# pangenome/povu

Measured on AMD Instinct MI355X. Metric: edges/sec decomposed (flubble+PVST), higher is better.
Workload: dtype u32

## Files before the change

include/povu_hip.h:

```cpp
#ifndef POVU_HIP_H
#define POVU_HIP_H

#include <stddef.h>
#include <stdint.h>

#ifdef __cplusplus
extern "C" {
#endif

#define POVU_HIP_NIL 0xFFFFFFFFu
#define POVU_SIDE_L 0
#define POVU_SIDE_R 1
#define POVU_TIP_NONE 0
#define POVU_TIP_L 1
#define POVU_TIP_R 2

typedef struct povu_hip_ctx povu_hip_ctx;
typedef struct povu_hip_forest povu_hip_forest;

int povu_hip_device_count(void);

povu_hip_ctx *povu_hip_create(int device, char *err, size_t errlen);
void povu_hip_destroy(povu_hip_ctx *ctx);
int povu_hip_release_workspace(povu_hip_ctx *ctx);
// ... 563 lines not shown
typedef struct {
	char name[48];
	double ms;
	uint32_t launches;
} povu_hip_stage_time;
int povu_hip_last_stage_times(const povu_hip_ctx *ctx, povu_hip_stage_time *out, int max);
typedef struct { char name[24]; int resident; uint64_t bytes; } povu_hip_arena_info;
int povu_hip_arena_report(const povu_hip_ctx *ctx, povu_hip_arena_info *out, int max);
uint32_t povu_hip_last_seq_redo(const povu_hip_ctx *ctx);
int povu_hip_last_black_only_classes(const povu_hip_ctx *ctx);
int povu_hip_last_narrow_counts(const povu_hip_ctx *ctx);
int povu_hip_last_prefix_records(const povu_hip_ctx *ctx);
uint64_t povu_hip_wide_repeats(const povu_hip_ctx *ctx);
int povu_hip_last_laminar_check_ran(const povu_hip_ctx *ctx);
int povu_hip_last_crossings(povu_hip_ctx *ctx, uint32_t out[2]);
uint64_t povu_hip_last_links_processed(const povu_hip_ctx *ctx);

int povu_hip_debug_components(povu_hip_ctx *ctx, uint32_t *comp_of, uint32_t *local_idx);
int povu_hip_debug_tree(povu_hip_ctx *ctx, uint32_t comp, uint32_t *n_tree, uint32_t *gid, uint8_t *typ,
			uint32_t *par, uint32_t *cls);
int povu_hip_debug_edge_ids(povu_hip_ctx *ctx, uint32_t comp, uint32_t *n_tree, uint32_t *tree_edge_id);
int povu_hip_debug_walk_words(povu_hip_ctx *ctx, uint32_t out[3]);
int povu_hip_debug_stack(povu_hip_ctx *ctx, uint32_t comp, uint32_t *n, uint32_t *tree_vtx, uint32_t *cls,
			 uint32_t *next_seen);

int povu_hip_debug_csr(povu_hip_ctx *ctx, uint32_t *off, uint32_t *adj, uint32_t *aoth, uint32_t *atwin, uint8_t *tip,
		       uint32_t words[4]);
#define POVU_HIP_ROWB_IDENTITY 1u
#define POVU_HIP_ROWB_SORT_FREE 2u
#define POVU_HIP_ROWB_LEAN_IDENTITY 4u
// ... 66 lines not shown
```

povu_amd/csrc/hip/common.hpp:

```cpp
#pragma once
#include <hip/hip_runtime.h>

#include "forest_wire.hpp"

#include <algorithm>
#include <cstdint>
#include <cstdio>
#include <cstring>
#include <stdexcept>
#include <string>
#include <vector>

#define POVU_NIL 0xFFFFFFFFu

__device__ __forceinline__ uint4 load4_unaligned(const unsigned *__restrict__ p)
{
	typedef unsigned v4a __attribute__((ext_vector_type(4), aligned(4)));
	const v4a v = *reinterpret_cast<const v4a *>(p);
	return make_uint4(v.x, v.y, v.z, v.w);
}

#define POVU_W2(v) "+v"((v).x), "+v"((v).y)
#define POVU_W4(v) "+v"((v).x), "+v"((v).y), "+v"((v).z), "+v"((v).w)
__device__ __forceinline__ void landed(uint32_t &a, uint32_t &b, uint32_t &c, uint32_t &d) { asm volatile("" : "+v"(a), "+v"(b), "+v"(c), "+v"(d)); }
__device__ __forceinline__ void landed(uint32_t &a, uint32_t &b, uint32_t &c, uint32_t &d, uint32_t &e)
{
	asm volatile("" : "+v"(a), "+v"(b), "+v"(c), "+v"(d), "+v"(e));
}
__device__ __forceinline__ void landed(uint2 &a, uint2 &b, uint2 &c, uint2 &d, uint32_t &e, uint32_t &f, uint32_t &g, uint32_t &h)
{
	asm volatile("" : POVU_W2(a), POVU_W2(b), POVU_W2(c), POVU_W2(d), "+v"(e), "+v"(f), "+v"(g), "+v"(h));
}
__device__ __forceinline__ void landed(uint4 &a, uint2 &b) { asm volatile("" : POVU_W4(a), POVU_W2(b)); }
__device__ __forceinline__ void landed(uint4 &a, uint4 &b, uint4 &c, uint4 &d) { asm volatile("" : POVU_W4(a), POVU_W4(b), POVU_W4(c), POVU_W4(d)); }
#define POVU_A2(a, W) W((a)[0]), W((a)[1])
#define POVU_A4(a, W) POVU_A2(a, W), W((a)[2]), W((a)[3])
#define POVU_A8(a, W) POVU_A4(a, W), W((a)[4]), W((a)[5]), W((a)[6]), W((a)[7])
#define POVU_W1(v) "+v"(v)
template <uint32_t N>
__device__ __forceinline__ void landed(uint32_t (&a)[N], uint32_t (&b)[N], uint32_t (&c)[N], uint32_t (&d)[N], uint32_t (&e)[N])
{
	static_assert(N == 2 || N == 4 || N == 8, "a batch of 2, 4 or 8");
	if constexpr (N == 2)
		asm volatile("" : POVU_A2(a, POVU_W1), POVU_A2(b, POVU_W1), POVU_A2(c, POVU_W1), POVU_A2(d, POVU_W1), POVU_A2(e, POVU_W1));
	else if constexpr (N == 4)
		asm volatile("" : POVU_A4(a, POVU_W1), POVU_A4(b, POVU_W1), POVU_A4(c, POVU_W1), POVU_A4(d, POVU_W1), POVU_A4(e, POVU_W1));
	else
		asm volatile("" : POVU_A8(a, POVU_W1), POVU_A8(b, POVU_W1), POVU_A8(c, POVU_W1), POVU_A8(d, POVU_W1), POVU_A8(e, POVU_W1));
// ... 563 lines not shown
```

povu_amd/csrc/hip/par_kernels.hip:

```cpp
#include "par_kernels.hpp"
#include "segtree.hpp"

#include <algorithm>
#include <cstdlib>
#include <type_traits>

namespace povu_hip
{

#define NIL POVU_NIL
static constexpr size_t PVST_STAGE_MIN = size_t(1) << 20;

__global__ void k_tcomp_vertices(uint32_t V, uint32_t T, const uint32_t *__restrict__ ckey, const uint32_t *__restrict__ voff,
				 uint32_t *__restrict__ t_comp)
{
	uint32_t i = BIDX * blockDim.x + threadIdx.x;
	if (i >= V)
		return;
	uint32_t c = ckey[i];
	t_comp[2 * i + c] = c;
	t_comp[2 * i + 1 + c] = c;
	if (i + 1 == voff[c + 1])
		t_comp[2 * i + 2 + c] = c;
	if (i == V - 1)
// ... 107 lines not shown
	__device__ __forceinline__ uint32_t operator()(uint32_t t) const
	{
		if (t_root)
			return t_root[t];
		uint32_t lo = 0, hi = C;
		while (hi - lo > 1) {
			const uint32_t mid = (lo + hi) >> 1;
			if (2 * voff[mid] + mid <= t)
				lo = mid;
			else
				hi = mid;
		}
		return 2 * voff[lo] + lo;
	}
};
__device__ __forceinline__ void capping_of(uint32_t v, const uint32_t *__restrict__ gsize, const uint32_t *__restrict__ hi0,
					   const uint4 *__restrict__ brec, const RootOf &root_of,
					   const SegTree &segA, uint32_t *__restrict__ cap_tgt,
					   uint8_t *__restrict__ capf, uint32_t *__restrict__ literal_rule_seen)
{
	const uint32_t end = v + gsize[v];
	uint32_t root = NIL;
	auto hi_of = [&](uint32_t c) {
		const uint32_t cs = max(gsize[c], 1u);
		if (bitrank(brec, c + cs) != bitrank(brec, c)) {
			if (root == NIL)
				root = root_of(v);
			return root;
		}
		if (cs <= 8) {
			uint32_t m = NIL;
			for (uint32_t k = c; k < c + cs; k++)
				m = min(m, hi0[k]);
			return m;
		}
		return seg_min(segA, c, c + cs);
	};
	uint32_t hi_1 = NIL, hi_child = NIL, lt_c[2] = {NIL, NIL}, lt_h[2] = {NIL, NIL};
	uint32_t second = NIL;
	for (uint32_t c = v + 1; c < end; c += max(gsize[c], 1u)) {
		const uint32_t h = hi_of(c);
		if (h < hi_1 || hi_child == NIL) {
			second = hi_1;
			hi_1 = h;
			hi_child = c;
		} else {
			second = min(second, h);
		}
		if (h < v) {
			if (lt_c[0] == NIL)
				lt_c[0] = c, lt_h[0] = h;
			else if (lt_c[1] == NIL)
				lt_c[1] = c, lt_h[1] = h;
		}
	}
	const uint32_t hi_2 = lt_c[0] != hi_child ? lt_h[0] : lt_h[1];
	if (hi_2 != (second < v ? second : NIL))
		*literal_rule_seen = 1u;
	if (hi_2 < hi0[v]) {
		cap_tgt[v] = hi_2;
		capf[v] = 1;
	}
}
static constexpr uint32_t HS_ITER = LIST_ITER, HS_VERTS = LIST_SPAN;
static_assert(TPB == (int)LIST_TPB, "append_in_order is written for workgroups of 256");
__global__ void __launch_bounds__(TPB) k_hi_simp(uint32_t T, const uint32_t *__restrict__ gsize, const uint4 *__restrict__ brec,
						  uint8_t *__restrict__ simp, uint8_t *__restrict__ hpf,
						  uint8_t *__restrict__ capf, uint32_t *__restrict__ br_list, uint32_t *__restrict__ n_br)
{
	const uint32_t B0 = BIDX * HS_VERTS;
	auto one = [&](uint32_t t, uint32_t sz, uint32_t br, uint32_t p0, uint32_t sz_next, uint32_t &sm, uint32_t &bch) {
		sm = (sz && br && bitrank(brec, t + sz) - p0 == 1) ? 1u : 0u;
		bch = (sz > 2 && t + 1 + max(sz_next, 1u) < t + sz) ? 1u : 0u;
	};
// ... 28 lines not shown
				simp[t] = (uint8_t)sm;
				if (t == T - 1)
					simp[T] = 0;
				if (hpf)
					hpf[t] = (uint8_t)sm;
				capf[t] = 0;
				b4 |= bch << (t - t0);
			}
		}
		bw |= (unsigned long long)b4 << (4 * it);
	}
	append_in_order(bw, B0, br_list, n_br);
}
__global__ void k_capping(const uint32_t *__restrict__ n_list, const uint32_t *__restrict__ list, const uint32_t *__restrict__ gsize,
			  const uint32_t *__restrict__ hi0, const uint4 *__restrict__ brec, const RootOf root_of, const SegTree segA,
			  uint32_t *__restrict__ cap_tgt, uint8_t *__restrict__ capf, uint32_t *__restrict__ literal_rule_seen)
{
	const uint32_t n = *n_list;
	for (uint32_t i = BIDX * blockDim.x + threadIdx.x; i < n; i += gridDim.x * blockDim.x)
		capping_of(list[i], gsize, hi0, brec, root_of, segA, cap_tgt, capf, literal_rule_seen);
}
static constexpr uint32_t BX_TILE = TPB;
__global__ void __launch_bounds__(TPB) k_flag_tile_counts(uint32_t T, const uint8_t *__restrict__ capf, const uint8_t *__restrict__ simp,
							   uint32_t *__restrict__ tcap, uint32_t *__restrict__ tsimp, uint32_t ntiles)
{
	const uint32_t e0 = (blockIdx.x * TPB + threadIdx.x) * 16u;
	uint32_t nc = 0, ns = 0;
	if (e0 + 16 <= T) {
		const uint4 a = *reinterpret_cast<const uint4 *>(capf + e0), b = *reinterpret_cast<const uint4 *>(simp + e0);
		const uint32_t wa[4] = {a.x, a.y, a.z, a.w}, wb[4] = {b.x, b.y, b.z, b.w};
#pragma unroll
		for (int k = 0; k < 4; k++)
#pragma unroll
			for (int q = 0; q < 4; q++) {
				nc += ((wa[k] >> (8 * q)) & 0xFFu) ? 1u : 0u;
// ... 153 lines not shown
	uint32_t i = BIDX * blockDim.x + threadIdx.x;
	if (i < n)
		dst[i] = src[idx[i]];
}
struct StackPlace {
	const uint32_t *voff, *soff, *shift;
	uint32_t *s_vtx;
};
template <bool BLACK, class PS, class BS>
__global__ void k_top_bracket(uint32_t n, const uint32_t *__restrict__ gsize, const uint32_t *__restrict__ gpar,
			      const uint32_t *__restrict__ mpre, const BS bstart,
			      const SegTree segB, const uint32_t *__restrict__ tgtR,
			      const PS psin, uint32_t *__restrict__ ckey, uint32_t *__restrict__ cval,
			      uint32_t *__restrict__ lsz, uint32_t *__restrict__ err, const uint32_t *__restrict__ rid,
			      uint32_t first_simp_id, uint8_t *__restrict__ hpf, const uint32_t *__restrict__ seg_comp,
			      const uint32_t *__restrict__ c_ntree, const StackPlace sp)
{
	const uint32_t q = BIDX * blockDim.x + threadIdx.x;
	if (q >= n)
		return;
	uint32_t v = n - 1 - q, c = 0;
	const uint32_t g = v;
	if (BLACK) {
		c = seg_comp[g];
		v = 2 * g + c + (c_ntree[c] & 1u) + 1;
	}
	uint32_t sz = gsize[v];
	if (sz == 0 || (!BLACK && gpar[v] == NIL)) {
		cval[q] = v;
		ckey[q] = NIL;
		if (!BLACK)
			lsz[v] = 0;
		return;
	}
	uint32_t at = v;
	if (BLACK) {
		at = sp.soff[c] + (g - sp.voff[c]) + sp.shift[g];
		sp.s_vtx[at] = v;
	}
	cval[q] = at;
	uint32_t m = mpre[v];
	uint32_t lo = bstart.at(m), hi = bstart.at(m + sz);
	const uint32_t live = (hi - lo) - (psin.at(v + sz) - psin.at(v));
	uint32_t i = NIL;
	if (live >= 1 && live <= 4) {
		const uint4 a = load4_unaligned(tgtR + (hi - live));
		const bool all = a.x < v && (live < 2 || a.y < v) && (live < 3 || a.z < v) && (live < 4 || a.w < v);
		if (all)
			i = hi - live;
	}
	if (i == NIL) {
		const uint32_t np = min(hi - lo, 4u);
		const uint4 a = load4_unaligned(tgtR + lo);
		if (np > 0 && a.x < v)
			i = lo;
		else if (np > 1 && a.y < v)
			i = lo + 1;
		else if (np > 2 && a.z < v)
			i = lo + 2;
		else if (np > 3 && a.w < v)
			i = lo + 3;
		if (i == NIL && lo + np < hi)
			i = seg_first_less(segB, lo + np, hi, v);
	}
	if (i == NIL) {
		atomicAdd(&err[PW_NO_BRACKET], 1u);
		ckey[q] = NIL;
		lsz[at] = 0;
		return;
	}
	lsz[at] = live;
	ckey[q] = i;
	if (hpf && rid[i] >= first_simp_id)
		hpf[v] |= 2;
}
template <bool BLACK>
__global__ void k_class_flags(uint32_t n, uint32_t V, const uint32_t *__restrict__ skey, const uint32_t *__restrict__ sval,
			      const uint32_t *__restrict__ lsz, const uint8_t *__restrict__ tf, uint8_t *__restrict__ flag,
			      uint32_t *__restrict__ dlt, uint32_t *__restrict__ mark)
{
	uint32_t q = BIDX * blockDim.x + threadIdx.x;
	if (!BLACK && q < V + 2)
		dlt[q] = 0;
	if (q >= n)
		return;
	uint32_t k = skey[q];
// ... 65 lines not shown
		return;
	const uint32_t p = lastb[q];
	if (!p)
		return;
	const uint32_t u = sval[q], d = sval[p - 1];
	if (gcls[u] != gcls[d])
		return;
	const uint32_t iu = sidx[u], id = sidx[d];
	ns[iu] = id;
	prev[id] = iu;
}

static constexpr uint32_t DF_OPENS = 1u, DF_SEEN = 2u;
__global__ void k_class_finish_black(uint32_t n, uint32_t S, const uint32_t *__restrict__ skey, const uint32_t *__restrict__ sval,
				     const uint32_t *__restrict__ lsz, uint8_t *__restrict__ flag, uint32_t *__restrict__ ns,
				     uint32_t *__restrict__ prev, bool write_prev, uint8_t *__restrict__ dflag)
{
	const uint32_t q0 = (BIDX * blockDim.x + threadIdx.x) * 4u;
	if (q0 == 0)
		dflag[S] = 0;
	if (q0 >= n)
		return;
	uint32_t K[6], U[6], L[6];
	if (q0 + 4 <= n) {
		const uint4 k4 = *reinterpret_cast<const uint4 *>(skey + q0), u4 = *reinterpret_cast<const uint4 *>(sval + q0);
		K[1] = k4.x, K[2] = k4.y, K[3] = k4.z, K[4] = k4.w;
		U[1] = u4.x, U[2] = u4.y, U[3] = u4.z, U[4] = u4.w;
	} else {
		for (uint32_t j = 1; j <= 4; j++) {
			K[j] = q0 + j - 1 < n ? skey[q0 + j - 1] : NIL;
			U[j] = q0 + j - 1 < n ? sval[q0 + j - 1] : 0u;
		}
	}
	K[0] = q0 ? skey[q0 - 1] : NIL, U[0] = q0 ? sval[q0 - 1] : 0u;
	K[5] = q0 + 4 < n ? skey[q0 + 4] : NIL, U[5] = q0 + 4 < n ? sval[q0 + 4] : 0u;
#pragma unroll
	for (int j = 0; j < 6; j++)
		L[j] = K[j] != NIL ? lsz[U[j]] : 0u;
	bool fresh[6];
	fresh[0] = true;
#pragma unroll
	for (int j = 1; j < 6; j++)
		fresh[j] = (q0 + j - 1 == 0) || K[j - 1] != K[j] || L[j - 1] != L[j];
	uint32_t fw = 0;
#pragma unroll
	for (int j = 1; j <= 4; j++) {
		const uint32_t q = q0 + j - 1;
		if (q >= n || K[j] == NIL)
			continue;
		const uint32_t u = U[j];
		fw |= (fresh[j] ? 1u : 0u) << (8 * (j - 1));
		const uint32_t nx = fresh[j] ? u : U[j - 1];
		ns[u] = nx;
		const bool seen = K[j + 1] != NIL && !fresh[j + 1];
		if (write_prev)
			prev[u] = seen ? U[j + 1] : NIL;
		dflag[u] = (uint8_t)(((u + 1 < nx) ? DF_OPENS : 0u) | (seen ? DF_SEEN : 0u));
	}
	if (q0 + 4 <= n) {
		*reinterpret_cast<uint32_t *>(flag + q0) = fw;
	} else {
		for (uint32_t j = 0; q0 + j < n; j++)
			flag[q0 + j] = (uint8_t)((fw >> (8 * j)) & 0xFFu);
	}
}
__global__ void k_class_ids_black(uint32_t n, const uint32_t *__restrict__ skey, const uint32_t *__restrict__ sval,
				  const uint8_t *__restrict__ fresh, const uint32_t *__restrict__ ps, uint32_t *__restrict__ s_cls)
{
	uint32_t q = BIDX * blockDim.x + threadIdx.x;
	if (q < n && skey[q] != NIL)
		s_cls[sval[q]] = ps[q] + fresh[q] - 1;
}
__global__ void k_cls_from_stack(uint32_t S, const uint32_t *__restrict__ s_vtx, const uint32_t *__restrict__ s_cls,
				 uint32_t *__restrict__ gcls)
{
	uint32_t i = BIDX * blockDim.x + threadIdx.x;
	if (i < S)
		gcls[s_vtx[i]] = s_cls[i];
}
__device__ __forceinline__ void laminar_check_one(uint32_t i, uint32_t p, const uint32_t *__restrict__ prev, const SegTree &segP,
						   uint8_t *__restrict__ xflag)
{
	if (p == NIL || p + 1 >= i)
		return;
	uint32_t lowest;
	if (i - p <= 9) {
// ... 513 lines not shown
	ParWs &pw;
	StageTimer &tm;
	hipStream_t s;
	const SideStream &side;
	PassTail &tail;
	const std::function<void *(size_t)> &alloc_result_block;
	const ClassViews v;
	const uint32_t C, V, T, S, n_processed;
	const int64_t dense_nb0;
	const bool dense;
	const bool want_hp;
	const bool lean;
	const bool narrow_oc, narrow_sc, narrow_ic;
	const int word_prefix;
	const bool rec_ps, rec_bs;
	bool black_only = false;
	const RootOf root_of;
	uint32_t NB0 = 0, ncap = 0, nsimp = 0, NB = 0, NC = 0;
	const uint32_t ntiles;
	uint32_t *extra = nullptr;
	HostScratch::Token extra_ready = 0;
	uint32_t *early = nullptr;
	HostScratch::Token early_ready = 0;
	bool use_side = false;

	ClassPass(const CompState &cs_, SeqWs &sw_, ParWs &pw_, uint32_t C_, uint32_t n_processed_, uint32_t n_stack, int64_t dense_nb0_,
		  const std::function<void *(size_t)> &alloc, StageTimer &tm_, hipStream_t s_, const SideStream &side_, PassTail &tail_)
		: cs(cs_), sw(sw_), pw(pw_), tm(tm_), s(s_), side(side_), tail(tail_), alloc_result_block(alloc), v(class_views(pw_)), C(C_),
		  V(sw_.V), T(2 * sw_.V + C_), S(n_stack), n_processed(n_processed_), dense_nb0(dense_nb0_), dense(dense_nb0_ >= 0),
		  want_hp(sw_.hairpins != nullptr), lean(dense && !want_hp), narrow_oc(dense && pw_.narrow_ordcnt),
		  narrow_sc(narrow_oc && pw_.narrow_srccnt), narrow_ic(narrow_sc && pw_.narrow_incnt),
		  word_prefix(getenv("POVU_HIP_WORD_PREFIX") ? atoi(getenv("POVU_HIP_WORD_PREFIX")) : 0), rec_ps(narrow_ic && word_prefix != 1 && word_prefix != 2),
		  rec_bs(narrow_sc && word_prefix != 1 && word_prefix != 3), root_of{lean ? nullptr : pw_.t_root, cs_.voff, C_},
		  ntiles((T + BX_TILE - 1) / BX_TILE)
	{
	}
	void scan(const uint32_t *in, uint32_t *out, size_t n) const { scan_exclusive_u32(in, out, n, pw.scan_tmp, pw.scan_tmp_bytes, s); }
	void scan8(const uint8_t *in, uint32_t *out, size_t n) const
	{
		scan_exclusive_u8(in, out, n, nullptr, nullptr, 0, pw.scan_tmp, pw.scan_tmp_bytes, s);
	}
	void scan8pair(const uint8_t *in0, uint32_t *out0, size_t n0, const uint8_t *in1, uint32_t *out1, size_t n1) const
	{
		scan_exclusive_u8(in0, out0, n0, in1, out1, n1, pw.scan_tmp, pw.scan_tmp_bytes, s);
	}
	uint4 *psin_rec() const { return reinterpret_cast<uint4 *>(pw.psin); }
	uint4 *bstart_rec() const { return reinterpret_cast<uint4 *>(v.bstart); }
	template <class F>
// ... 60 lines not shown
	seg_build(pw.segA, pw.hi0, T, s);
	if (P.narrow_ic)
		scan_exclusive_diff_u8_u8(pw.ordcnt8, pw.incnt8, v.pscov, (size_t)T + 1, pw.scan_tmp, pw.scan_tmp_bytes, s);
	else if (P.narrow_oc)
		scan_exclusive_diff_u8_u32(pw.ordcnt8, pw.incnt, v.pscov, (size_t)T + 1, pw.scan_tmp, pw.scan_tmp_bytes, s);
	else if (P.dense)
		scan_exclusive_diff_u32(pw.lsz, pw.incnt, v.pscov, (size_t)T + 1, pw.scan_tmp, pw.scan_tmp_bytes, s);
	else
		P.scan(pw.cov, v.pscov, (size_t)T + 1);
	KLAUNCH(k_bridge_flags, dim3(nblk(((size_t)T / 256 + 1) * 64)), dim3(TPB), 0, s, T, pw.gsize, P.sw.t_flags, v.pscov, v.brec);
	bitrank_build(v.brec, (size_t)T / 64 + 1, v.brec_cnt, pw.scan_tmp, pw.scan_tmp_bytes, s);
	uint32_t *n_br = pw.err + PW_N_BRIDGE;
	KLAUNCH(k_hi_simp, dim3((unsigned)(((size_t)T + HS_VERTS - 1) / HS_VERTS)), dim3(TPB), 0, s, T, pw.gsize, v.brec, v.simp, P.want_hp ? pw.hpf : nullptr, v.capf, v.br_list,
		n_br);
	KLAUNCH(k_capping, dim3(std::min<unsigned>(nblk(T / 8 + 1), 16384)), dim3(TPB), 0, s, n_br, v.br_list, pw.gsize, pw.hi0, v.brec, P.root_of,
		pw.segA, pw.cap_tgt, v.capf, pw.err + PW_LITERAL_RULE);
	KLAUNCH(k_flag_tile_counts, dim3((ntiles + 1 + 15) / 16 + 1), dim3(TPB), 0, s, T, v.capf, v.simp, v.tcap, v.tsimp, ntiles);
	scan_exclusive_u32_pair(v.tsimp, v.tsimp, (size_t)ntiles + 1, v.tcap, v.tcap, (size_t)ntiles + 1, pw.scan_tmp, pw.scan_tmp_bytes, s);
	if (!P.narrow_ic)
		publish_extra(P);
}

static bool place_brackets(ClassPass &P)
{
	ParWs &pw = P.pw;
	const ClassViews &v = P.v;
	hipStream_t s = P.s;
	const uint32_t T = P.T;
	auto bracket_extra = [&](auto *ordcnt, auto *sc, auto *ic) {
		using OC = std::remove_const_t<std::remove_pointer_t<decltype(ordcnt)>>;
		using SC = std::remove_pointer_t<decltype(sc)>;
// ... 79 lines not shown
{
	ParWs &pw = P.pw;
	const ClassViews &v = P.v;
	const CompState &cs = P.cs;
	hipStream_t s = P.s;
	const uint32_t V = P.V, NC = P.NC;
	uint32_t *sdl = pw.dlt;
	if (pw.sdl_filled && P.dense) {
		sdl = pw.sdl;
	} else {
		HIP_CHECK(hipMemsetAsync(pw.dlt, 0, ((size_t)V + 2) * 4, s));
		LAUNCH(k_shift_delta, V, s, V, cs.ckey, P.sw.c_ntree, pw.gsize, pw.dlt);
	}
	scan_inclusive_u32(sdl, v.shift_ps, (size_t)V + 1, pw.scan_tmp, pw.scan_tmp_bytes, s);
	const StackPlace sp{cs.voff, pw.soff, v.shift_ps, pw.s_vtx};
	P.with_prefix_views([&](auto ps, auto bs) {
		LAUNCH((k_top_bracket<true, decltype(ps), decltype(bs)>), NC, s, NC, pw.gsize, pw.gpar, pw.mpre, bs, pw.segB, pw.tgtR, ps, v.ck,
		       pw.vals_t, pw.lsz, pw.err, pw.b_val2, P.NB0 + P.ncap, nullptr, cs.ckey, P.sw.c_ntree, sp);
	});
	sort_pairs_u32(v.ck, v.ck2, pw.vals_t, pw.vals_t2, NC, bits_for((uint64_t)P.NB + 1), pw.sort_tmp, pw.sort_tmp_bytes, s);
	P.tm.end(30 + 2 * 22);
	P.tm.begin("par_stack");
	LAUNCH(k_class_finish_black, std::max<size_t>(((size_t)NC + 3) / 4, 1), s, NC, P.S, v.ck2, pw.vals_t2, pw.lsz, v.cflag, pw.ns, pw.prev,
	       pw.check_laminar, v.dflag);
	P.tm.end(1);
	P.tm.begin("par_next_seen");
	P.tm.end(0);
	pw.gcls_valid = false;
	pw.s_cls_valid = false;
}

static void classes_all_vertices(ClassPass &P)
{
	ParWs &pw = P.pw;
	const ClassViews &v = P.v;
	const CompState &cs = P.cs;
	const SeqWs &sw = P.sw;
	hipStream_t s = P.s;
	const uint32_t V = P.V, T = P.T, NC = P.NC;
	const StackPlace none{nullptr, nullptr, nullptr, nullptr};
	P.with_prefix_views([&](auto ps, auto bs) {
		LAUNCH((k_top_bracket<false, decltype(ps), decltype(bs)>), NC, s, NC, pw.gsize, pw.gpar, pw.mpre, bs, pw.segB, pw.tgtR, ps, v.ck,
		       pw.vals_t, pw.lsz, pw.err, pw.b_val2, P.NB0 + P.ncap, P.want_hp ? pw.hpf : nullptr, nullptr, nullptr, none);
	});
	sort_pairs_u32(v.ck, v.ck2, pw.vals_t, pw.vals_t2, NC, bits_for((uint64_t)P.NB + 1), pw.sort_tmp, pw.sort_tmp_bytes, s);
	LAUNCH(k_class_flags<false>, std::max<size_t>(NC, (size_t)V + 2), s, NC, V, v.ck2, pw.vals_t2, pw.lsz, sw.t_flags, v.cflag, pw.dlt,
	       v.mark);
	P.scan8(v.cflag, v.cps, (size_t)NC + 1);
	LAUNCH(k_class_scatter, NC, s, NC, v.ck2, pw.vals_t2, v.cflag, v.cps, pw.gcls);
	pw.gcls_valid = true;
	pw.s_cls_valid = true;
	P.tm.end(30 + 2 * 22);

	P.tm.begin("par_stack");
	LAUNCH(k_shift_delta, V, s, V, cs.ckey, sw.c_ntree, pw.gsize, pw.dlt);
	P.scan(pw.dlt, pw.dlt_ps, (size_t)V + 1);
	LAUNCH(k_stack_emit, V, s, V, cs.ckey, sw.c_ntree, cs.voff, pw.soff, pw.dlt, pw.dlt_ps, pw.gsize, pw.gcls, pw.s_vtx, pw.s_cls,
	       pw.topi, pw.ns, pw.prev);
// ... 154 lines not shown
	else
		classes_all_vertices(P);
	stack_directories(P);
	laminar_and_levels(P);
	emit_and_copy(P);
	return true;
}

static void stack_class_ids(ParWs &pw, hipStream_t s)
{
	if (pw.s_cls_valid)
		return;
	const uint32_t V = pw.V;
	const ClassViews v = class_views(pw);
	scan_exclusive_u8(v.cflag, v.cps, (size_t)V + 1, nullptr, nullptr, 0, pw.scan_tmp, pw.scan_tmp_bytes, s);
	LAUNCH(k_class_ids_black, V, s, V, v.ck2, pw.vals_t2, v.cflag, v.cps, pw.s_cls);
	pw.s_cls_valid = true;
}
void classes_to_tree_space(ParWs &pw, hipStream_t s)
{
	if (pw.gcls_valid)
		return;
	stack_class_ids(pw, s);
	HIP_CHECK(hipMemsetAsync(pw.gcls, 0xFF, (size_t)pw.T * 4, s));
	if (pw.n_stack)
		LAUNCH(k_cls_from_stack, pw.n_stack, s, pw.n_stack, pw.s_vtx, pw.s_cls, pw.gcls);
	pw.gcls_valid = true;
}

void export_parallel_stack(const CompState &cs, SeqWs &sw, ParWs &pw, hipStream_t s)
{
	stack_class_ids(pw, s);
// ... 7 lines not shown
```

povu_amd/csrc/hip/par_kernels.hpp:

```cpp
#pragma once
#include "common.hpp"
#include "graph_kernels.hpp"
#include "seq_kernels.hpp"

#include <functional>

namespace povu_hip
{

struct SegTree {
	uint32_t *tree = nullptr;
	const uint32_t *val = nullptr;
	uint32_t P = 1;
	static constexpr uint32_t BLK = 16;
	static uint32_t pow2(size_t n)
	{
		uint32_t p = 1;
		while (p < n)
			p <<= 1;
		return p;
	}
	static size_t tree_words(size_t n) { return 2 * (size_t)pow2((n + BLK - 1) / BLK + 1); }
};

enum PassWord : uint32_t {
	PW_NO_BRACKET = 0,
	PW_FOREST_SIZE = 2,
	PW_N_OVER = 4,
	PW_LITERAL_RULE = 5,
	PW_NB0 = 6,
	PW_POOL_TOP = 7,
	PW_WALK_POOL = 8,
	PW_N_ENTRY = 9,
	PW_N_BRIDGE = 10,
	PW_N_X = 11,
	PW_N_CROSSED = 12,
	PW_RANK_OVF = 13,
	PW_INCNT_OVF = 14,
	PASS_WORDS = 16
};

__device__ __forceinline__ uint32_t incnt_add(uint32_t *incnt, uint32_t t) { return atomicAdd(&incnt[t], 1u); }
__device__ __forceinline__ uint32_t incnt_add(uint8_t *incnt, uint32_t t)
{
	const unsigned sh = 8u * (t & 3u);
	return (atomicAdd(reinterpret_cast<uint32_t *>(incnt + (t & ~3u)), 1u << sh) >> sh) & 0xFFu;
}
__device__ __forceinline__ void incnt_take_back(uint8_t *incnt, uint32_t t)
{
	atomicSub(reinterpret_cast<uint32_t *>(incnt + (t & ~3u)), 1u << (8u * (t & 3u)));
}

struct PassSummary {
	enum Err : uint32_t { NO_BRACKET = 0, WALK_POOL = 1, FOREST_SIZE = 2, SPARE = 3, ERR_WORDS = 4 };
	uint32_t C;
// ... 5 lines not shown
	__host__ __device__ uint32_t &status(uint32_t c) const { return w[ERR_WORDS + (size_t)C + c]; }
	__host__ __device__ uint32_t &npvst(uint32_t c) const { return w[ERR_WORDS + 2 * (size_t)C + c]; }
	__host__ __device__ uint32_t &nbry(uint32_t c) const { return w[ERR_WORDS + 3 * (size_t)C + c]; }
	__host__ __device__ uint32_t &doff(uint32_t c) const { return w[ERR_WORDS + 4 * (size_t)C + c]; }
	__host__ __device__ uint32_t total() const { return doff(C); }
};

struct ParWs {
	HostScratch *host;
	uint32_t V, E, C, T;
	bool all_vertex_classes = false;
	bool check_laminar = false;
	bool laminar_checked = false;
	bool black_only_used = false;
	int prefix_records = 0;
	bool s_cls_valid = false;
	bool gcls_valid = false;
	uint32_t *t_comp, *t_root, *gpar, *gsize;
	uint32_t *hi0, *cov, *psA, *psB, *flagC, *psC;
	uint8_t *f8a, *f8b, *f8c, *f8d;
	uint32_t *cap_tgt, *mpre, *dlt, *dlt_ps, *incnt, *psin, *topi, *lsz, *gcls;
	uint8_t *ordcnt8, *srccnt8;
	bool narrow_ordcnt = false, narrow_srccnt = false;
	uint8_t *incnt8;
	bool narrow_incnt = false;
	uint32_t *sdl;
	bool sdl_filled = false;
	uint32_t *vals_t, *vals_t2;
	uint32_t *keys_t, *keys_t2;
	uint32_t *dbo;
// ... 47 lines not shown
	bool sorted_brackets = true;
	bool hairpins = true;
	bool walk_inline = true;
};
size_t par_workspace_bytes(size_t V, size_t E, size_t Cmax, int groups = 3, const StageWsOpts &o = StageWsOpts{});
void par_carve(Arena &ar, ParWs &pw, size_t V, size_t E, size_t Cmax, int groups = 3, const StageWsOpts &o = StageWsOpts{});

static constexpr int64_t NB0_ON_DEVICE = int64_t(1) << 40;
bool run_parallel_dg(const CompState &cs, SeqWs &sw, ParWs &pw, uint32_t C, uint32_t n_processed, uint32_t n_stack,
		     int64_t dense_nb0, const std::function<void *(size_t)> &alloc_result_block, StageTimer &tm, hipStream_t s,
		     const SideStream &side, PassTail &tail);

void run_parallel_hairpins(const CompState &cs, SeqWs &sw, ParWs &pw, uint32_t C, StageTimer &tm, hipStream_t s);

void classes_to_tree_space(ParWs &pw, hipStream_t s);
void export_parallel_stack(const CompState &cs, SeqWs &sw, ParWs &pw, hipStream_t s);

void pass_summary(const SeqWs &sw, const ParWs *pw, uint32_t C, uint32_t *host_out, hipStream_t s);

}
```

povu_amd/csrc/hip/povu_hip.hip:

```cpp
#include "context.hpp"

#include <algorithm>
#include <atomic>
#include <cstdlib>
#include <memory>
#include <mutex>
#include <numeric>

#include <fcntl.h>
#include <sys/mman.h>
#include <unistd.h>

using namespace povu_hip;

PinnedPool::~PinnedPool()
{
	for (auto &b : free_blocks)
		if (b.seg < 0)
			(void)hipHostFree(b.p);
	for (auto &sg : segments) {
		(void)hipHostUnregister(sg.p);
		(void)munmap(sg.p, sg.cap);
		(void)shm_unlink(segment_name(shared_tag, sg.seg).c_str());
	}
// ... 1530 lines not shown

extern "C" int povu_hip_last_crossings(povu_hip_ctx *ctx, uint32_t out[2])
{
	if (!ctx || !out)
		return 1;
	out[0] = out[1] = 0;
	if (!ctx->last.valid || ctx->last.plan.all_seq || !ctx->pw.laminar_checked)
		return 0;
	ctx->quiesce();
	if (hipSetDevice(ctx->device) != hipSuccess)
		return 2;
	static_assert(PW_N_CROSSED == PW_N_X + 1, "the two crossing words are copied as a pair");
	return hipMemcpy(out, ctx->pw.err + PW_N_X, 8, hipMemcpyDeviceToHost) == hipSuccess ? 0 : 2;
}

extern "C" int povu_hip_last_laminar_check_ran(const povu_hip_ctx *ctx)
{
	return ctx && ctx->last.valid && !ctx->last.plan.all_seq && ctx->pw.laminar_checked ? 1 : 0;
}
```

povu_amd/hip.py:

```python
from __future__ import annotations

import ctypes as C
import os
from dataclasses import dataclass
from typing import Dict, List, Optional

import numpy as np

_HERE = os.path.dirname(os.path.abspath(__file__))


class HipUnavailable(RuntimeError):
    pass


class GuardBandError(RuntimeError):
    """A device-wide primitive wrote outside its output (raised by its unit-test hook, which guards every output)."""


SCAN_SUM, SCAN_MAX, SCAN_U64, SCAN_U8, SCAN_DIFF, SCAN_XOR_PAIR, SCAN_XOR_U128, SCAN_DIFF_U8, SCAN_MIXED_PAIR, SCAN_DIFF_U8_U8, SCAN_INCLUSIVE = range(11)
SCAN_IN_PLACE, SCAN_N_DEV = 0x100, 0x200
SEG_MIN, SEG_FIRST_LESS, SEG_LAST_LESS = range(3)


# ... 423 lines not shown
    l.povu_hip_componetize.restype = C.POINTER(_Components)
    l.povu_hip_componetize.argtypes = [C.c_void_p, C.c_char_p, C.c_size_t]
    l.povu_hip_components_free.restype = None
    l.povu_hip_components_free.argtypes = [C.POINTER(_Components)]
    l.povu_hip_debug_tree.restype = C.c_int
    l.povu_hip_debug_tree.argtypes = [C.c_void_p, C.c_uint32, C.POINTER(C.c_uint32), C.c_void_p, C.c_void_p,
                                      C.c_void_p, C.c_void_p]
    l.povu_hip_last_narrow_counts.restype = C.c_int
    l.povu_hip_last_narrow_counts.argtypes = [C.c_void_p]
    l.povu_hip_wide_repeats.restype = C.c_uint64
    l.povu_hip_wide_repeats.argtypes = [C.c_void_p]
    l.povu_hip_last_black_only_classes.restype = C.c_int
    l.povu_hip_last_black_only_classes.argtypes = [C.c_void_p]
    l.povu_hip_last_crossings.restype = C.c_int
    l.povu_hip_last_crossings.argtypes = [C.c_void_p, C.POINTER(C.c_uint32)]
    l.povu_hip_last_laminar_check_ran.restype = C.c_int
    l.povu_hip_last_laminar_check_ran.argtypes = [C.c_void_p]
    l.povu_hip_debug_edge_ids.restype = C.c_int
    l.povu_hip_debug_edge_ids.argtypes = [C.c_void_p, C.c_uint32, C.POINTER(C.c_uint32), C.c_void_p]
    l.povu_hip_debug_walk_words.restype = C.c_int
    l.povu_hip_debug_walk_words.argtypes = [C.c_void_p, C.POINTER(C.c_uint32)]
    l.povu_hip_debug_stack.restype = C.c_int
    l.povu_hip_debug_stack.argtypes = [C.c_void_p, C.c_uint32, C.POINTER(C.c_uint32), C.c_void_p, C.c_void_p,
                                       C.c_void_p]
    l.povu_hip_version.restype = C.c_char_p
    l.povu_hip_debug_scan.restype = C.c_int
    l.povu_hip_debug_scan.argtypes = [C.c_void_p, C.c_int, C.c_void_p, C.c_void_p, C.c_size_t, C.c_void_p, C.c_void_p,
                                      C.c_size_t]
    l.povu_hip_debug_sort.restype = C.c_int
    l.povu_hip_debug_sort.argtypes = [C.c_void_p, C.c_void_p, C.c_void_p, C.c_size_t, C.c_uint, C.c_void_p, C.c_void_p]
# ... 1321 lines not shown
    def last_prefix_records(self) -> int:
        return int(self._lib.povu_hip_last_prefix_records(self._ctx))

    def wide_repeat_count(self) -> int:
        return int(self._lib.povu_hip_wide_repeats(self._ctx))

    def last_black_only_classes(self) -> bool:
        return bool(self._lib.povu_hip_last_black_only_classes(self._ctx))

    def last_crossings(self):
        o = (C.c_uint32 * 2)()
        if self._lib.povu_hip_last_crossings(self._ctx, o) != 0:
            raise RuntimeError("povu_hip_last_crossings failed")
        return int(o[0]), int(o[1])

    def last_laminar_check_ran(self) -> bool:
        return bool(self._lib.povu_hip_last_laminar_check_ran(self._ctx))

    def debug_edge_ids(self, comp: int):
        n = C.c_uint32(0)
        rc = self._lib.povu_hip_debug_edge_ids(self._ctx, comp, C.byref(n), None)
        if rc != 0:
            raise RuntimeError("no parallel-tree state" if rc == 3 else "no decompose state")
        ids = np.zeros(n.value, dtype=np.uint32)
        if self._lib.povu_hip_debug_edge_ids(self._ctx, comp, C.byref(n), ids.ctypes.data) != 0:
            raise RuntimeError("povu_hip_debug_edge_ids failed")
        return ids

    def debug_walk_words(self):
        o = (C.c_uint32 * 3)()
# ... 79 lines not shown
```

Measured before the change: 3.565 billion.

## Pack bracket size into sort value bits and batch capping child loads

In the black-only path, the live bracket count is packed into the spare high bits of the sorted value word. The class-finish kernel can then read sizes directly from the sorted values, and only gathers from lsz when a size saturates the field. This cuts the random lsz scatter and gather traffic, at the cost of extra bit manipulation and a fallback path for large counts. Separately, the capping kernel prefetches the first two children's gsize, bit-rank records and hi0 windows in one batch so their loads overlap. A debug API is added to report the field width and how many entries saturate.

```diff
diff --git a/include/povu_hip.h b/include/povu_hip.h
--- a/include/povu_hip.h
+++ b/include/povu_hip.h
@@ -601,6 +601,7 @@
 uint64_t povu_hip_wide_repeats(const povu_hip_ctx *ctx);
 int povu_hip_last_laminar_check_ran(const povu_hip_ctx *ctx);
 int povu_hip_last_crossings(povu_hip_ctx *ctx, uint32_t out[2]);
+int povu_hip_last_lsz_field(povu_hip_ctx *ctx, uint32_t out[2]);
 uint64_t povu_hip_last_links_processed(const povu_hip_ctx *ctx);
 
 int povu_hip_debug_components(povu_hip_ctx *ctx, uint32_t *comp_of, uint32_t *local_idx);
diff --git a/povu_amd/csrc/hip/common.hpp b/povu_amd/csrc/hip/common.hpp
--- a/povu_amd/csrc/hip/common.hpp
+++ b/povu_amd/csrc/hip/common.hpp
@@ -27,11 +27,21 @@
 {
 	asm volatile("" : "+v"(a), "+v"(b), "+v"(c), "+v"(d), "+v"(e));
 }
+__device__ __forceinline__ void landed(uint32_t &a, uint32_t &b, uint32_t &c, uint32_t &d, uint32_t &e, uint32_t &f)
+{
+	asm volatile("" : "+v"(a), "+v"(b), "+v"(c), "+v"(d), "+v"(e), "+v"(f));
+}
 __device__ __forceinline__ void landed(uint2 &a, uint2 &b, uint2 &c, uint2 &d, uint32_t &e, uint32_t &f, uint32_t &g, uint32_t &h)
 {
 	asm volatile("" : POVU_W2(a), POVU_W2(b), POVU_W2(c), POVU_W2(d), "+v"(e), "+v"(f), "+v"(g), "+v"(h));
 }
+__device__ __forceinline__ void landed(uint4 &a) { asm volatile("" : POVU_W4(a)); }
 __device__ __forceinline__ void landed(uint4 &a, uint2 &b) { asm volatile("" : POVU_W4(a), POVU_W2(b)); }
+__device__ __forceinline__ void landed(uint32_t &a, uint4 &b, uint4 &c, uint4 &d) { asm volatile("" : "+v"(a), POVU_W4(b), POVU_W4(c), POVU_W4(d)); }
+__device__ __forceinline__ void landed(uint32_t &a, uint32_t &b, uint32_t &c, uint4 &d, uint4 &e, uint4 &f)
+{
+	asm volatile("" : "+v"(a), "+v"(b), "+v"(c), POVU_W4(d), POVU_W4(e), POVU_W4(f));
+}
 __device__ __forceinline__ void landed(uint4 &a, uint4 &b, uint4 &c, uint4 &d) { asm volatile("" : POVU_W4(a), POVU_W4(b), POVU_W4(c), POVU_W4(d)); }
 #define POVU_A2(a, W) W((a)[0]), W((a)[1])
 #define POVU_A4(a, W) POVU_A2(a, W), W((a)[2]), W((a)[3])
diff --git a/povu_amd/csrc/hip/par_kernels.hip b/povu_amd/csrc/hip/par_kernels.hip
--- a/povu_amd/csrc/hip/par_kernels.hip
+++ b/povu_amd/csrc/hip/par_kernels.hip
@@ -145,20 +145,33 @@
 		return 2 * voff[lo] + lo;
 	}
 };
+__device__ __forceinline__ uint32_t bitrank_in(const uint4 &r, uint32_t x)
+{
+	const unsigned long long bits = (unsigned long long)r.x | ((unsigned long long)r.y << 32);
+	return r.z + (uint32_t)__popcll(bits & ((1ull << (x & 63u)) - 1ull));
+}
+__device__ __forceinline__ uint32_t min_of_first(const uint4 &a, const uint4 &b, uint32_t n)
+{
+	uint32_t m = a.x;
+	m = min(m, n > 1 ? a.y : NIL), m = min(m, n > 2 ? a.z : NIL), m = min(m, n > 3 ? a.w : NIL);
+	m = min(m, n > 4 ? b.x : NIL), m = min(m, n > 5 ? b.y : NIL), m = min(m, n > 6 ? b.z : NIL), m = min(m, n > 7 ? b.w : NIL);
+	return m;
+}
 __device__ __forceinline__ void capping_of(uint32_t v, const uint32_t *__restrict__ gsize, const uint32_t *__restrict__ hi0,
 					   const uint4 *__restrict__ brec, const RootOf &root_of,
 					   const SegTree &segA, uint32_t *__restrict__ cap_tgt,
-					   uint8_t *__restrict__ capf, uint32_t *__restrict__ literal_rule_seen)
-{
-	const uint32_t end = v + gsize[v];
+					   uint8_t *__restrict__ capf, uint32_t *__restrict__ literal_rule_seen, uint32_t hi0_words)
+{
 	uint32_t root = NIL;
+	auto root_once = [&]() __attribute__((always_inline)) {
+		if (root == NIL)
+			root = root_of(v);
+		return root;
+	};
 	auto hi_of = [&](uint32_t c) {
 		const uint32_t cs = max(gsize[c], 1u);
-		if (bitrank(brec, c + cs) != bitrank(brec, c)) {
-			if (root == NIL)
-				root = root_of(v);
-			return root;
-		}
+		if (bitrank(brec, c + cs) != bitrank(brec, c))
+			return root_once();
 		if (cs <= 8) {
 			uint32_t m = NIL;
 			for (uint32_t k = c; k < c + cs; k++)
@@ -167,10 +180,9 @@
 		}
 		return seg_min(segA, c, c + cs);
 	};
-	uint32_t hi_1 = NIL, hi_child = NIL, lt_c[2] = {NIL, NIL}, lt_h[2] = {NIL, NIL};
+	uint32_t hi_1 = NIL, hi_child = NIL, lt_c0 = NIL, lt_c1 = NIL, lt_h0 = NIL, lt_h1 = NIL;
 	uint32_t second = NIL;
-	for (uint32_t c = v + 1; c < end; c += max(gsize[c], 1u)) {
-		const uint32_t h = hi_of(c);
+	auto take = [&](uint32_t c, uint32_t h) __attribute__((always_inline)) {
 		if (h < hi_1 || hi_child == NIL) {
 			second = hi_1;
 			hi_1 = h;
@@ -178,17 +190,42 @@
 		} else {
 			second = min(second, h);
 		}
-		if (h < v) {
-			if (lt_c[0] == NIL)
-				lt_c[0] = c, lt_h[0] = h;
-			else if (lt_c[1] == NIL)
-				lt_c[1] = c, lt_h[1] = h;
-		}
-	}
-	const uint32_t hi_2 = lt_c[0] != hi_child ? lt_h[0] : lt_h[1];
+		const bool f0 = h < v && lt_c0 == NIL, f1 = h < v && !f0 && lt_c1 == NIL;
+		lt_c0 = f0 ? c : lt_c0, lt_h0 = f0 ? h : lt_h0;
+		lt_c1 = f1 ? c : lt_c1, lt_h1 = f1 ? h : lt_h1;
+	};
+	uint32_t c = v + 1, end, hv;
+	if (c + 8 <= hi0_words) {
+		uint32_t szv = gsize[v], g1 = gsize[c];
+		hv = hi0[v];
+		uint4 r1 = brec[c >> 6], a1 = load4_unaligned(hi0 + c), b1 = load4_unaligned(hi0 + c + 4);
+		landed(szv, hv, g1, r1, a1, b1);
+		end = v + szv;
+		const uint32_t cs1 = max(g1, 1u), c2 = c + cs1;
+		if (c2 + 8 <= hi0_words) {
+			uint32_t g2 = gsize[c2];
+			uint4 r2 = brec[c2 >> 6], a2 = load4_unaligned(hi0 + c2), b2 = load4_unaligned(hi0 + c2 + 4);
+			landed(g2, r2, a2, b2);
+			const uint32_t cs2 = max(g2, 1u), c3 = c2 + cs2;
+			uint4 r3 = r2;
+			landed(r3);
+			if ((c3 >> 6) != (c2 >> 6))
+				r3 = brec[c3 >> 6];
+			const uint32_t k1 = bitrank_in(r1, c), k2 = bitrank_in(r2, c2), k3 = bitrank_in(r3, c3);
+			take(c, k2 != k1 ? root_once() : cs1 <= 8 ? min_of_first(a1, b1, cs1) : seg_min(segA, c, c2));
+			take(c2, k3 != k2 ? root_once() : cs2 <= 8 ? min_of_first(a2, b2, cs2) : seg_min(segA, c2, c3));
+			c = c3;
+		}
+	} else {
+		end = v + gsize[v];
+		hv = hi0[v];
+	}
+	for (; c < end; c += max(gsize[c], 1u))
+		take(c, hi_of(c));
+	const uint32_t hi_2 = lt_c0 != hi_child ? lt_h0 : lt_h1;
 	if (hi_2 != (second < v ? second : NIL))
 		*literal_rule_seen = 1u;
-	if (hi_2 < hi0[v]) {
+	if (hi_2 < hv) {
 		cap_tgt[v] = hi_2;
 		capf[v] = 1;
 	}
@@ -247,11 +284,12 @@
 }
 __global__ void k_capping(const uint32_t *__restrict__ n_list, const uint32_t *__restrict__ list, const uint32_t *__restrict__ gsize,
 			  const uint32_t *__restrict__ hi0, const uint4 *__restrict__ brec, const RootOf root_of, const SegTree segA,
-			  uint32_t *__restrict__ cap_tgt, uint8_t *__restrict__ capf, uint32_t *__restrict__ literal_rule_seen)
+			  uint32_t *__restrict__ cap_tgt, uint8_t *__restrict__ capf, uint32_t *__restrict__ literal_rule_seen,
+			  uint32_t hi0_words)
 {
 	const uint32_t n = *n_list;
 	for (uint32_t i = BIDX * blockDim.x + threadIdx.x; i < n; i += gridDim.x * blockDim.x)
-		capping_of(list[i], gsize, hi0, brec, root_of, segA, cap_tgt, capf, literal_rule_seen);
+		capping_of(list[i], gsize, hi0, brec, root_of, segA, cap_tgt, capf, literal_rule_seen, hi0_words);
 }
 static constexpr uint32_t BX_TILE = TPB;
 __global__ void __launch_bounds__(TPB) k_flag_tile_counts(uint32_t T, const uint8_t *__restrict__ capf, const uint8_t *__restrict__ simp,
@@ -435,7 +473,7 @@
 			      const PS psin, uint32_t *__restrict__ ckey, uint32_t *__restrict__ cval,
 			      uint32_t *__restrict__ lsz, uint32_t *__restrict__ err, const uint32_t *__restrict__ rid,
 			      uint32_t first_simp_id, uint8_t *__restrict__ hpf, const uint32_t *__restrict__ seg_comp,
-			      const uint32_t *__restrict__ c_ntree, const StackPlace sp)
+			      const uint32_t *__restrict__ c_ntree, const StackPlace sp, const LszField lf)
 {
 	const uint32_t q = BIDX * blockDim.x + threadIdx.x;
 	if (q >= n)
@@ -459,7 +497,6 @@
 		at = sp.soff[c] + (g - sp.voff[c]) + sp.shift[g];
 		sp.s_vtx[at] = v;
 	}
-	cval[q] = at;
 	uint32_t m = mpre[v];
 	uint32_t lo = bstart.at(m), hi = bstart.at(m + sz);
 	const uint32_t live = (hi - lo) - (psin.at(v + sz) - psin.at(v));
@@ -487,10 +524,19 @@
 	if (i == NIL) {
 		atomicAdd(&err[PW_NO_BRACKET], 1u);
 		ckey[q] = NIL;
-		lsz[at] = 0;
-		return;
-	}
-	lsz[at] = live;
+		cval[q] = at;
+		if (!BLACK)
+			lsz[at] = 0;
+		return;
+	}
+	if (BLACK) {
+		cval[q] = lf.pack(at, live);
+		if (live >= lf.lmax)
+			lsz[at] = live;
+	} else {
+		cval[q] = at;
+		lsz[at] = live;
+	}
 	ckey[q] = i;
 	if (hpf && rid[i] >= first_simp_id)
 		hpf[v] |= 2;
@@ -586,7 +632,7 @@
 static constexpr uint32_t DF_OPENS = 1u, DF_SEEN = 2u;
 __global__ void k_class_finish_black(uint32_t n, uint32_t S, const uint32_t *__restrict__ skey, const uint32_t *__restrict__ sval,
 				     const uint32_t *__restrict__ lsz, uint8_t *__restrict__ flag, uint32_t *__restrict__ ns,
-				     uint32_t *__restrict__ prev, bool write_prev, uint8_t *__restrict__ dflag)
+				     uint32_t *__restrict__ prev, bool write_prev, uint8_t *__restrict__ dflag, const LszField lf)
 {
 	const uint32_t q0 = (BIDX * blockDim.x + threadIdx.x) * 4u;
 	if (q0 == 0)
@@ -594,6 +640,8 @@
 	if (q0 >= n)
 		return;
 	uint32_t K[6], U[6], L[6];
+	const uint32_t qa = q0 ? q0 - 1 : 0u, qz = min(q0 + 4, n - 1);
+	uint32_t ka = skey[qa], ua = sval[qa], kz = skey[qz], uz = sval[qz];
 	if (q0 + 4 <= n) {
 		const uint4 k4 = *reinterpret_cast<const uint4 *>(skey + q0), u4 = *reinterpret_cast<const uint4 *>(sval + q0);
 		K[1] = k4.x, K[2] = k4.y, K[3] = k4.z, K[4] = k4.w;
@@ -604,11 +652,27 @@
 			U[j] = q0 + j - 1 < n ? sval[q0 + j - 1] : 0u;
 		}
 	}
-	K[0] = q0 ? skey[q0 - 1] : NIL, U[0] = q0 ? sval[q0 - 1] : 0u;
-	K[5] = q0 + 4 < n ? skey[q0 + 4] : NIL, U[5] = q0 + 4 < n ? sval[q0 + 4] : 0u;
+	landed(ka, ua, kz, uz);
+	K[0] = q0 ? ka : NIL, U[0] = q0 ? ua : 0u;
+	K[5] = q0 + 4 < n ? kz : NIL, U[5] = q0 + 4 < n ? uz : 0u;
+	bool sat[6], any_sat = false;
 #pragma unroll
-	for (int j = 0; j < 6; j++)
-		L[j] = K[j] != NIL ? lsz[U[j]] : 0u;
+	for (int j = 0; j < 6; j++) {
+		L[j] = K[j] != NIL ? lf.size(U[j]) : 0u;
+		U[j] = lf.index(U[j]);
+		sat[j] = K[j] != NIL && L[j] == lf.lmax;
+		any_sat |= sat[j];
+	}
+	if (__any(any_sat)) {
+		uint32_t t[6];
+#pragma unroll
+		for (int j = 0; j < 6; j++)
+			t[j] = gather_if(sat[j], lsz, U[j], q0);
+		landed(t[0], t[1], t[2], t[3], t[4], t[5]);
+#pragma unroll
+		for (int j = 0; j < 6; j++)
+			L[j] = sat[j] ? t[j] : L[j];
+	}
 	bool fresh[6];
 	fresh[0] = true;
 #pragma unroll
@@ -637,11 +701,21 @@
 	}
 }
 __global__ void k_class_ids_black(uint32_t n, const uint32_t *__restrict__ skey, const uint32_t *__restrict__ sval,
-				  const uint8_t *__restrict__ fresh, const uint32_t *__restrict__ ps, uint32_t *__restrict__ s_cls)
+				  const uint8_t *__restrict__ fresh, const uint32_t *__restrict__ ps, uint32_t *__restrict__ s_cls,
+				  const LszField lf)
 {
 	uint32_t q = BIDX * blockDim.x + threadIdx.x;
 	if (q < n && skey[q] != NIL)
-		s_cls[sval[q]] = ps[q] + fresh[q] - 1;
+		s_cls[lf.index(sval[q])] = ps[q] + fresh[q] - 1;
+}
+__global__ void k_count_saturated(uint32_t n, const uint32_t *__restrict__ skey, const uint32_t *__restrict__ sval, const LszField lf,
+				  uint32_t *__restrict__ count)
+{
+	const uint32_t q = BIDX * blockDim.x + threadIdx.x;
+	const bool sat = q < n && skey[q] != NIL && lf.size(sval[q]) == lf.lmax;
+	const unsigned long long sm = __ballot(sat);
+	if (sm && (threadIdx.x & 63u) == 0)
+		atomicAdd(count, (uint32_t)__popcll(sm));
 }
 __global__ void k_cls_from_stack(uint32_t S, const uint32_t *__restrict__ s_vtx, const uint32_t *__restrict__ s_cls,
 				 uint32_t *__restrict__ gcls)
@@ -1185,6 +1259,7 @@
 	const bool narrow_oc, narrow_sc, narrow_ic;
 	const int word_prefix;
 	const bool rec_ps, rec_bs;
+	const unsigned lsz_cap;
 	bool black_only = false;
 	const RootOf root_of;
 	uint32_t NB0 = 0, ncap = 0, nsimp = 0, NB = 0, NC = 0;
@@ -1202,7 +1277,8 @@
 		  want_hp(sw_.hairpins != nullptr), lean(dense && !want_hp), narrow_oc(dense && pw_.narrow_ordcnt),
 		  narrow_sc(narrow_oc && pw_.narrow_srccnt), narrow_ic(narrow_sc && pw_.narrow_incnt),
 		  word_prefix(getenv("POVU_HIP_WORD_PREFIX") ? atoi(getenv("POVU_HIP_WORD_PREFIX")) : 0), rec_ps(narrow_ic && word_prefix != 1 && word_prefix != 2),
-		  rec_bs(narrow_sc && word_prefix != 1 && word_prefix != 3), root_of{lean ? nullptr : pw_.t_root, cs_.voff, C_},
+		  rec_bs(narrow_sc && word_prefix != 1 && word_prefix != 3),
+		  lsz_cap(getenv("POVU_HIP_LSZ_FIELD") ? (unsigned)std::min(std::max(atoi(getenv("POVU_HIP_LSZ_FIELD")), 0), (int)LSZ_FIELD_CAP) : LSZ_FIELD_CAP), root_of{lean ? nullptr : pw_.t_root, cs_.voff, C_},
 		  ntiles((T + BX_TILE - 1) / BX_TILE)
 	{
 	}
@@ -1293,7 +1369,7 @@
 	KLAUNCH(k_hi_simp, dim3((unsigned)(((size_t)T + HS_VERTS - 1) / HS_VERTS)), dim3(TPB), 0, s, T, pw.gsize, v.brec, v.simp, P.want_hp ? pw.hpf : nullptr, v.capf, v.br_list,
 		n_br);
 	KLAUNCH(k_capping, dim3(std::min<unsigned>(nblk(T / 8 + 1), 16384)), dim3(TPB), 0, s, n_br, v.br_list, pw.gsize, pw.hi0, v.brec, P.root_of,
-		pw.segA, pw.cap_tgt, v.capf, pw.err + PW_LITERAL_RULE);
+		pw.segA, pw.cap_tgt, v.capf, pw.err + PW_LITERAL_RULE, T + 2);
 	KLAUNCH(k_flag_tile_counts, dim3((ntiles + 1 + 15) / 16 + 1), dim3(TPB), 0, s, T, v.capf, v.simp, v.tcap, v.tsimp, ntiles);
 	scan_exclusive_u32_pair(v.tsimp, v.tsimp, (size_t)ntiles + 1, v.tcap, v.tcap, (size_t)ntiles + 1, pw.scan_tmp, pw.scan_tmp_bytes, s);
 	if (!P.narrow_ic)
@@ -1403,15 +1479,16 @@
 	}
 	scan_inclusive_u32(sdl, v.shift_ps, (size_t)V + 1, pw.scan_tmp, pw.scan_tmp_bytes, s);
 	const StackPlace sp{cs.voff, pw.soff, v.shift_ps, pw.s_vtx};
+	const LszField lf = pw.lsz_field = lsz_field(P.S, P.lsz_cap);
 	P.with_prefix_views([&](auto ps, auto bs) {
 		LAUNCH((k_top_bracket<true, decltype(ps), decltype(bs)>), NC, s, NC, pw.gsize, pw.gpar, pw.mpre, bs, pw.segB, pw.tgtR, ps, v.ck,
-		       pw.vals_t, pw.lsz, pw.err, pw.b_val2, P.NB0 + P.ncap, nullptr, cs.ckey, P.sw.c_ntree, sp);
+		       pw.vals_t, pw.lsz, pw.err, pw.b_val2, P.NB0 + P.ncap, nullptr, cs.ckey, P.sw.c_ntree, sp, lf);
 	});
 	sort_pairs_u32(v.ck, v.ck2, pw.vals_t, pw.vals_t2, NC, bits_for((uint64_t)P.NB + 1), pw.sort_tmp, pw.sort_tmp_bytes, s);
 	P.tm.end(30 + 2 * 22);
 	P.tm.begin("par_stack");
 	LAUNCH(k_class_finish_black, std::max<size_t>(((size_t)NC + 3) / 4, 1), s, NC, P.S, v.ck2, pw.vals_t2, pw.lsz, v.cflag, pw.ns, pw.prev,
-	       pw.check_laminar, v.dflag);
+	       pw.check_laminar, v.dflag, lf);
 	P.tm.end(1);
 	P.tm.begin("par_next_seen");
 	P.tm.end(0);
@@ -1428,9 +1505,10 @@
 	hipStream_t s = P.s;
 	const uint32_t V = P.V, T = P.T, NC = P.NC;
 	const StackPlace none{nullptr, nullptr, nullptr, nullptr};
+	pw.lsz_field = LszField{0, 32, 0};
 	P.with_prefix_views([&](auto ps, auto bs) {
 		LAUNCH((k_top_bracket<false, decltype(ps), decltype(bs)>), NC, s, NC, pw.gsize, pw.gpar, pw.mpre, bs, pw.segB, pw.tgtR, ps, v.ck,
-		       pw.vals_t, pw.lsz, pw.err, pw.b_val2, P.NB0 + P.ncap, P.want_hp ? pw.hpf : nullptr, nullptr, nullptr, none);
+		       pw.vals_t, pw.lsz, pw.err, pw.b_val2, P.NB0 + P.ncap, P.want_hp ? pw.hpf : nullptr, nullptr, nullptr, none, pw.lsz_field);
 	});
 	sort_pairs_u32(v.ck, v.ck2, pw.vals_t, pw.vals_t2, NC, bits_for((uint64_t)P.NB + 1), pw.sort_tmp, pw.sort_tmp_bytes, s);
 	LAUNCH(k_class_flags<false>, std::max<size_t>(NC, (size_t)V + 2), s, NC, V, v.ck2, pw.vals_t2, pw.lsz, sw.t_flags, v.cflag, pw.dlt,
@@ -1615,8 +1693,17 @@
 	const uint32_t V = pw.V;
 	const ClassViews v = class_views(pw);
 	scan_exclusive_u8(v.cflag, v.cps, (size_t)V + 1, nullptr, nullptr, 0, pw.scan_tmp, pw.scan_tmp_bytes, s);
-	LAUNCH(k_class_ids_black, V, s, V, v.ck2, pw.vals_t2, v.cflag, v.cps, pw.s_cls);
+	LAUNCH(k_class_ids_black, V, s, V, v.ck2, pw.vals_t2, v.cflag, v.cps, pw.s_cls, pw.lsz_field);
 	pw.s_cls_valid = true;
+}
+uint32_t count_saturated(ParWs &pw, hipStream_t s)
+{
+	if (!pw.black_only_used)
+		return 0;
+	const ClassViews v = class_views(pw);
+	HIP_CHECK(hipMemsetAsync(pw.err + PW_LSZ_SAT, 0, 4, s));
+	LAUNCH(k_count_saturated, pw.V, s, pw.V, v.ck2, pw.vals_t2, pw.lsz_field, pw.err + PW_LSZ_SAT);
+	return pw.host->read_u32(pw.err + PW_LSZ_SAT, s);
 }
 void classes_to_tree_space(ParWs &pw, hipStream_t s)
 {
diff --git a/povu_amd/csrc/hip/par_kernels.hpp b/povu_amd/csrc/hip/par_kernels.hpp
--- a/povu_amd/csrc/hip/par_kernels.hpp
+++ b/povu_amd/csrc/hip/par_kernels.hpp
@@ -37,8 +37,35 @@
 	PW_N_CROSSED = 12,
 	PW_RANK_OVF = 13,
 	PW_INCNT_OVF = 14,
+	PW_LSZ_SAT = 15,
 	PASS_WORDS = 16
 };
+
+struct LszField {
+	unsigned w, abits;
+	uint32_t lmax;
+	__host__ __device__ constexpr uint32_t mask() const { return 0xFFFFFFFFu >> w; }
+	__host__ __device__ constexpr uint32_t pack(uint32_t at, uint32_t live) const { return at | (((live < lmax ? live : lmax) << 1) << (abits - 1)); }
+	__host__ __device__ constexpr uint32_t index(uint32_t u) const { return u & mask(); }
+	__host__ __device__ constexpr uint32_t size(uint32_t u) const { return (u >> 1) >> (abits - 1); }
+};
+static constexpr unsigned LSZ_FIELD_CAP = 8;
+constexpr LszField lsz_field(uint64_t S, unsigned cap = LSZ_FIELD_CAP)
+{
+	unsigned b = 1;
+	while (b < 32 && (uint64_t(1) << b) <= S)
+		b++;
+	const unsigned w = 32 - b < cap ? 32 - b : cap;
+	return LszField{w, 32 - w, (uint32_t(1) << w) - 1};
+}
+static_assert(lsz_field(1).w == 8 && lsz_field(1).abits == 24 && lsz_field(1).lmax == 255, "the cap");
+static_assert(lsz_field((1u << 24) - 1).w == 8 && lsz_field(1u << 24).w == 7 && lsz_field(1u << 24).abits == 25, "S = 2^24");
+static_assert(lsz_field((1u << 27) - 1).w == 5 && lsz_field(1u << 27).w == 4 && lsz_field(1u << 27).lmax == 15, "S = 2^27 - 1, 2^27");
+static_assert(lsz_field(1u << 29).w == 2 && lsz_field(1u << 29).mask() == 0x3FFFFFFFu, "S = 2^29");
+static_assert(lsz_field(0xFFFFFFFFull).w == 0 && lsz_field(0xFFFFFFFFull).lmax == 0 && lsz_field(0xFFFFFFFFull).mask() == 0xFFFFFFFFu, "S = 2^32 - 1: no field");
+static_assert(lsz_field(0xFFFFFFFFull).pack(0xFFFFFFFEu, 7) == 0xFFFFFFFEu && lsz_field(0xFFFFFFFFull).size(0xFFFFFFFEu) == 0, "no field: the bare index");
+static_assert(lsz_field(1u << 24, 3).w == 3 && lsz_field(1u << 29, 3).w == 2 && lsz_field(5, 0).w == 0, "a lower cap");
+static_assert(lsz_field(1u << 27).pack((1u << 27) - 1, 99) == 0xF7FFFFFFu && lsz_field(1u << 27).index(0xF7FFFFFFu) == (1u << 27) - 1 && lsz_field(1u << 27).size(0xF7FFFFFFu) == 15, "the largest index under a saturated size");
 
 __device__ __forceinline__ uint32_t incnt_add(uint32_t *incnt, uint32_t t) { return atomicAdd(&incnt[t], 1u); }
 __device__ __forceinline__ uint32_t incnt_add(uint8_t *incnt, uint32_t t)
@@ -74,6 +101,7 @@
 	bool laminar_checked = false;
 	bool black_only_used = false;
 	int prefix_records = 0;
+	LszField lsz_field{0, 32, 0};
 	bool s_cls_valid = false;
 	bool gcls_valid = false;
 	uint32_t *t_comp, *t_root, *gpar, *gsize;
@@ -151,6 +179,7 @@
 void run_parallel_hairpins(const CompState &cs, SeqWs &sw, ParWs &pw, uint32_t C, StageTimer &tm, hipStream_t s);
 
 void classes_to_tree_space(ParWs &pw, hipStream_t s);
+uint32_t count_saturated(ParWs &pw, hipStream_t s);
 void export_parallel_stack(const CompState &cs, SeqWs &sw, ParWs &pw, hipStream_t s);
 
 void pass_summary(const SeqWs &sw, const ParWs *pw, uint32_t C, uint32_t *host_out, hipStream_t s);
diff --git a/povu_amd/csrc/hip/povu_hip.hip b/povu_amd/csrc/hip/povu_hip.hip
--- a/povu_amd/csrc/hip/povu_hip.hip
+++ b/povu_amd/csrc/hip/povu_hip.hip
@@ -1568,6 +1568,25 @@
 	return hipMemcpy(out, ctx->pw.err + PW_N_X, 8, hipMemcpyDeviceToHost) == hipSuccess ? 0 : 2;
 }
 
+extern "C" int povu_hip_last_lsz_field(povu_hip_ctx *ctx, uint32_t out[2])
+{
+	if (!ctx || !out)
+		return 1;
+	out[0] = out[1] = 0;
+	if (!ctx->last.valid || ctx->last.plan.all_seq || !ctx->pw.black_only_used)
+		return 0;
+	ctx->quiesce();
+	if (hipSetDevice(ctx->device) != hipSuccess)
+		return 2;
+	try {
+		out[0] = ctx->pw.lsz_field.w;
+		out[1] = count_saturated(ctx->pw, ctx->stream);
+	} catch (const std::exception &) {
+		return 2;
+	}
+	return 0;
+}
+
 extern "C" int povu_hip_last_laminar_check_ran(const povu_hip_ctx *ctx)
 {
 	return ctx && ctx->last.valid && !ctx->last.plan.all_seq && ctx->pw.laminar_checked ? 1 : 0;
diff --git a/povu_amd/hip.py b/povu_amd/hip.py
--- a/povu_amd/hip.py
+++ b/povu_amd/hip.py
@@ -461,6 +461,8 @@
     l.povu_hip_last_black_only_classes.argtypes = [C.c_void_p]
     l.povu_hip_last_crossings.restype = C.c_int
     l.povu_hip_last_crossings.argtypes = [C.c_void_p, C.POINTER(C.c_uint32)]
+    l.povu_hip_last_lsz_field.restype = C.c_int
+    l.povu_hip_last_lsz_field.argtypes = [C.c_void_p, C.POINTER(C.c_uint32)]
     l.povu_hip_last_laminar_check_ran.restype = C.c_int
     l.povu_hip_last_laminar_check_ran.argtypes = [C.c_void_p]
     l.povu_hip_debug_edge_ids.restype = C.c_int
@@ -1812,6 +1814,12 @@
             raise RuntimeError("povu_hip_last_crossings failed")
         return int(o[0]), int(o[1])
 
+    def last_lsz_field(self):
+        o = (C.c_uint32 * 2)()
+        if self._lib.povu_hip_last_lsz_field(self._ctx, o) != 0:
+            raise RuntimeError("povu_hip_last_lsz_field failed")
+        return int(o[0]), int(o[1])
+
     def last_laminar_check_ran(self) -> bool:
         return bool(self._lib.povu_hip_last_laminar_check_ran(self._ctx))
 
```

After: 3.604 billion (median of 6 runs). +1.1%, better.
